# lmb-freiburg/flownet2

Measured on AMD Instinct MI355X. Metric: image-pairs/sec FlowNetC forward at 448x320, higher is better.
Workload: dtype f32

## Files before the change

### flownet2_amd/_lib.py

```python
from __future__ import annotations

import ctypes as C
import os

_HERE = os.path.dirname(os.path.abspath(__file__))
SO_PATH = os.path.join(_HERE, "libflownet2_hip.so")

EXPORTS = [
    "fn2_version", "fn2_last_error_string",
    "fn2_correlation_out_shape", "fn2_correlation_workspace_bytes", "fn2_correlation_forward", "fn2_correlation_forward_fused", "fn2_correlation_backward",
    "fn2_correlation1d_out_shape", "fn2_correlation1d_forward", "fn2_correlation1d_backward",
    "fn2_flow_warp_forward", "fn2_flow_warp_forward_slices", "fn2_flow_warp_backward_workspace_bytes", "fn2_flow_warp_backward",
    "fn2_resample_forward", "fn2_resample_forward_slices",
    "fn2_l1loss_workspace_bytes", "fn2_l1loss_forward", "fn2_l1loss_backward",
    "fn2_l1loss_multi_workspace_bytes", "fn2_l1loss_multi_sync_bytes", "fn2_l1loss_forward_multi", "fn2_l1loss_backward_multi",
    "fn2_channel_norm_forward", "fn2_channel_norm_forward_slices", "fn2_channel_norm_backward",
    "fn2_downsample_forward",
    "fn2_downsample_forward_multi",
    "fn2_predict_flow_conv_workspace_bytes", "fn2_predict_flow_conv_forward", "fn2_upsample_flow_deconv_forward", "fn2_upsample_flow_deconv_forward_into",
    "fn2_predict_flow_conv_backward_supported", "fn2_predict_flow_conv_backward_workspace_bytes", "fn2_predict_flow_conv_backward", "fn2_upsample_flow_deconv_backward_workspace_bytes", "fn2_upsample_flow_deconv_backward",
    "fn2_bias_leaky_relu_forward", "fn2_scale_shift_forward", "fn2_bias_leaky_relu_backward_workspace_bytes", "fn2_bias_leaky_relu_backward", "fn2_bias_leaky_relu_backward_slices", "fn2_bias_leaky_relu_backward_slices2",
    "fn2_conv_k7s2_relu_supported", "fn2_conv_k7s2_relu_forward",
    "fn2_conv_k7s2_wgrad_supported", "fn2_conv_k7s2_wgrad_ksplit", "fn2_conv_k7s2_wgrad_workspace_bytes", "fn2_conv_k7s2_wgrad",
    "fn2_conv_mfma_supported", "fn2_conv_mfma_packed_floats", "fn2_conv_mfma_pack_weights", "fn2_conv_mfma_pack_weights_view", "fn2_conv_mfma_forward",
    "fn2_conv_mfma_num_variants", "fn2_debug_set_conv_variant",
    "fn2_caffemodel_index", "fn2_caffemodel_read_blob", "fn2_hdf5_index", "fn2_hdf5_read_float",
    "fn2_conv_wino_supported", "fn2_conv_wino_packed_floats", "fn2_conv_wino_pack_weights", "fn2_conv_wino_forward",
    "fn2_conv_wino_num_variants", "fn2_debug_set_wino_variant",
    "fn2_conv_plane_supported", "fn2_conv_plane_ksplit", "fn2_conv_plane_workspace_bytes", "fn2_conv_plane_forward",
    "fn2_conv_plane_k_supported", "fn2_conv_plane_k_ksplit", "fn2_conv_plane_k_workspace_bytes", "fn2_conv_plane_k_forward",
    "fn2_conv_plane_num_variants", "fn2_debug_set_plane_variant", "fn2_debug_set_plane_ksplit", "fn2_set_batch_invariant", "fn2_get_batch_invariant",
    "fn2_deconv_plane_supported", "fn2_deconv_plane_ksplit", "fn2_deconv_plane_workspace_bytes", "fn2_deconv_plane_packed_floats",
    "fn2_deconv_plane_pack_weights", "fn2_deconv_plane_pack_weights_k", "fn2_deconv_plane_forward",
    "fn2_tconv_supported", "fn2_tconv_forward", "fn2_tconv_num_variants", "fn2_debug_set_tconv_variant",
    "fn2_debug_set_wgrad_buffers", "fn2_debug_set_wgrad_chunk", "fn2_conv_wgrad_supported", "fn2_conv_wgrad_ksplit", "fn2_conv_wgrad_workspace_bytes", "fn2_conv_wgrad",
    "fn2_conv_bf16x3_supported", "fn2_conv_bf16x3_num_variants", "fn2_debug_set_conv_bf16x3_variant",
    "fn2_conv_route", "fn2_conv_packed_weight_floats", "fn2_conv_pack_weights", "fn2_conv_workspace_bytes", "fn2_conv_forward",
    "fn2_deconv_route", "fn2_deconv_packed_weight_floats", "fn2_deconv_pack_weights", "fn2_deconv_workspace_bytes", "fn2_deconv_forward",
    "fn2_conv_backward_data_route", "fn2_conv_backward_data_packed_weight_floats", "fn2_conv_backward_data_pack_workspace_bytes",
    "fn2_conv_backward_data_pack_weights", "fn2_conv_backward_data_workspace_bytes", "fn2_conv_backward_data_workspace_bytes_with_room", "fn2_conv_backward_data_computed_channels", "fn2_conv_backward_data",
    "fn2_conv_backward_data_masked_supported", "fn2_conv_backward_data_masked", "fn2_conv_backward_weights_bias_fused", "fn2_conv_backward_weights_bias",
    "fn2_conv_backward_weights_supported", "fn2_conv_backward_weights_workspace_bytes", "fn2_conv_backward_weights", "fn2_conv_backward_bias",
    "fn2_im2col_forward", "fn2_col2im_bias_relu_forward", "fn2_col2im_bias_relu_forward_into",
    "fn2_datum_parse", "fn2_datum_float_data", "fn2_datum_serialize",
    "fn2_custom_data_sample_bytes", "fn2_custom_data_encode_sample", "fn2_custom_data_stage_records", "fn2_custom_data_decode_forward",
    "fn2_augmentation_matrix", "fn2_flow_augmentation_forward",
    "fn2_data_augmentation_workspace_bytes", "fn2_data_augmentation_forward",
]


class Fn2Error(RuntimeError):

    def __init__(self, status: int, message: str):
        super().__init__(f"[fn2 status {status}] {message}")
# ... 121 lines not shown
    L.fn2_debug_set_conv_variant.argtypes = [i]
    L.fn2_conv_wino_supported.argtypes = [i] * 5
    L.fn2_conv_wino_packed_floats.argtypes = [i, i]
    L.fn2_conv_wino_packed_floats.restype = sz
    L.fn2_conv_wino_pack_weights.argtypes = [fp, fp, i, i, vp]
    L.fn2_conv_wino_forward.argtypes = [fp, fp, fp, fp] + [i] * 11 + [C.c_float, vp]
    L.fn2_debug_set_wino_variant.argtypes = [i]
    L.fn2_conv_plane_supported.argtypes = [i] * 7
    L.fn2_conv_plane_ksplit.argtypes = [i] * 7
    L.fn2_conv_plane_workspace_bytes.argtypes = [i] * 7
    L.fn2_conv_plane_workspace_bytes.restype = sz
    L.fn2_conv_plane_forward.argtypes = [fp, fp, fp, fp] + [i] * 12 + [C.c_float, vp, sz, vp]
    L.fn2_conv_k7s2_wgrad_supported.argtypes = [i] * 5
    L.fn2_conv_k7s2_wgrad_ksplit.argtypes = [i] * 5
    L.fn2_conv_k7s2_wgrad_workspace_bytes.argtypes = [i] * 5
    L.fn2_conv_k7s2_wgrad_workspace_bytes.restype = sz
    L.fn2_conv_k7s2_wgrad.argtypes = [fp, fp, fp] + [i] * 6 + [vp, sz, vp]
    L.fn2_conv_plane_k_supported.argtypes = [i] * 8
    L.fn2_conv_plane_k_ksplit.argtypes = [i] * 8
    L.fn2_conv_plane_k_workspace_bytes.argtypes = [i] * 8
    L.fn2_conv_plane_k_workspace_bytes.restype = sz
    L.fn2_conv_plane_k_forward.argtypes = [fp, fp, fp, fp] + [i] * 13 + [C.c_float, vp, sz, vp]
    L.fn2_debug_set_plane_variant.argtypes = [i]
    L.fn2_debug_set_plane_ksplit.argtypes = [i]
    L.fn2_set_batch_invariant.argtypes = [i]
    L.fn2_get_batch_invariant.argtypes = []
    L.fn2_tconv_supported.argtypes = [i] * 8
    L.fn2_tconv_forward.argtypes = [fp, fp, fp, fp] + [i] * 14 + [C.c_float, vp]
    L.fn2_debug_set_tconv_variant.argtypes = [i]
    L.fn2_debug_set_wgrad_buffers.argtypes = [i]
    L.fn2_debug_set_wgrad_chunk.argtypes = [i]
    L.fn2_conv_wgrad_supported.argtypes = [i] * 10
    L.fn2_conv_wgrad_ksplit.argtypes = [i] * 10
    L.fn2_conv_wgrad_workspace_bytes.argtypes = [i] * 10
    L.fn2_conv_wgrad_workspace_bytes.restype = sz
    L.fn2_conv_wgrad.argtypes = [fp, fp, fp] + [i] * 15 + [vp, sz, vp]
    L.fn2_deconv_plane_supported.argtypes = [i] * 5
    L.fn2_deconv_plane_ksplit.argtypes = [i] * 5
    L.fn2_deconv_plane_workspace_bytes.argtypes = [i] * 5
    L.fn2_deconv_plane_workspace_bytes.restype = sz
    L.fn2_deconv_plane_packed_floats.argtypes = [i, i]
    L.fn2_deconv_plane_packed_floats.restype = sz
    L.fn2_deconv_plane_pack_weights.argtypes = [fp, fp, i, i, vp]
    L.fn2_deconv_plane_pack_weights_k.argtypes = [fp, fp, i, i, i, vp]
    L.fn2_deconv_plane_forward.argtypes = [fp, fp, fp, fp] + [i] * 10 + [C.c_float, vp, sz, vp]
    L.fn2_caffemodel_index.argtypes = [vp, sz, C.POINTER(CaffemodelEntry), i, C.POINTER(C.c_int)]
# ... 75 lines not shown
```

### flownet2_amd/csrc/conv_plane.hip

```cpp
#include "mfma_tile.hpp"

namespace fn2 {
namespace cp {

using namespace mfma;

constexpr int kNPR = 12;
constexpr int kLdsBytes = 160 * 1024;
constexpr int kSpare = 8;

struct Args {
  const float* in; const float* wp; const float* bias; float* out; float* part;
  int N, Cin, Hin, Win, in_ctot, in_c0;
  int Cout, Hout, Wout, out_ctot, out_c0;
  int pad;
  int P;
  int Wp;
  int img;
  int npb;
  int nig;
  int ng;
  int ksplit;
  int units;
  int ksteps;
  size_t class_stride;
  int rs, cs, wr;
  int band;
  int cap;
  int slots_c, npr;
  int buf;
  unsigned mP, mW, mrs;
  unsigned total;
  float slope; int relu;
};

template <int MODE_, int S_, int MW_, int NP_, int WM_, int WN_, int CQ_, int VEC_, int KS_ = 3>
struct Cfg {
  static constexpr int MODE = MODE_, S = S_, MW = MW_, NP = NP_, WM = WM_, WN = WN_, CQ = CQ_, VEC = VEC_, KS = KS_;
  static constexpr int NCLS = MODE == 1 ? 4 : 1;
  static constexpr int NW = NCLS * WM * WN, THREADS = 64 * NW;
  static constexpr int TAP = MODE == 1 ? 2 : KS;
  static constexpr int PADL = VEC == 4 ? 4 : (KS_ == 5 ? 2 : 1);
  static constexpr int KSC = CQ * TAP * TAP;
  static constexpr int NBUFA = KS_ == 5 ? 5 : (KSC % 9 == 0 && KSC > 9) ? 9 : (KSC % 8 == 0) ? 8 : (KSC % 4 == 0) ? 4 : 3;
  static constexpr int CAP = 16 * NP * WN;
  static_assert(KSC % NBUFA == 0, "ring phase must repeat per chunk");
  static_assert(NBUFA - 1 <= kSpare, "prefetch distance");
  static_assert(MODE == 0 || S == 1, "the deconvolution reads its input at stride 1");
  static_assert(KS == 3 || ((KS == 4 || KS == 5) && MODE == 0 && S == 2), "tap classes: 3x3 / 1, 3x3 / 2, 4x4 / 2, 5x5 / 2");
};

__device__ __forceinline__ int fastdiv(int q, int d, unsigned m) { return d == 1 ? q : (int)__umulhi((unsigned)q, m); }
inline unsigned magic_for(int d) { return d <= 1 ? 0u : (unsigned)(((1ull << 32) + (unsigned)d - 1) / (unsigned)d); }

template <class K>
__device__ __forceinline__ void stage_chunk(__amdgpu_buffer_rsrc_t rs, const unsigned (&voff)[kNPR], const Args& a, unsigned dst, int wave,
                                            unsigned chunk_off, unsigned plane_bytes, unsigned img_bytes, int nimg) {
  const int planes = nimg * 4 * K::CQ;
  const int last = a.slots_c - 64;
  for (int pl = wave; pl < planes; pl += K::NW) {
    const int il = pl / (4 * K::CQ), ch = pl % (4 * K::CQ);
    const unsigned soff = __builtin_amdgcn_readfirstlane(chunk_off + (unsigned)il * img_bytes + (unsigned)ch * plane_bytes);
    const unsigned d0 = __builtin_amdgcn_readfirstlane(dst + 4u * (unsigned)(pl * a.cs));
#pragma unroll
    for (int j = 0; j < kNPR; ++j) {
      if (j < a.npr) {
        const int s0 = 64 * j < last ? 64 * j : last;
        __builtin_amdgcn_raw_ptr_buffer_load_lds(rs, (lds_ptr_t)(uintptr_t)(d0 + 4u * K::VEC * (unsigned)s0), 4 * K::VEC, voff[j], soff, 0, 0);
      }
    }
  }
}

template <class K>
__global__ void __launch_bounds__(K::THREADS)
conv_plane(Args a) {
  extern __shared__ __attribute__((aligned(16))) float smem[];
  constexpr int S = K::S, MW = K::MW, NP = K::NP, TAP = K::TAP;
  unsigned t;
  if (!xcd_task(blockIdx.x, a.total, t)) return;
  const int g = __builtin_amdgcn_readfirstlane((int)(t % a.ng)); t /= a.ng;
  const int pb = __builtin_amdgcn_readfirstlane((int)(t % a.npb)); t /= a.npb;
  const int ig = __builtin_amdgcn_readfirstlane((int)(t % a.nig));
  const int kp = __builtin_amdgcn_readfirstlane((int)(t / a.nig));

  const int tid = threadIdx.x, lane = tid & 63;
  const int wave = __builtin_amdgcn_readfirstlane(tid >> 6);
  const int cls = wave % K::NCLS, w2 = wave / K::NCLS;
  const int py = cls >> 1, px = cls & 1;
  const int wm = w2 % K::WM, wn = w2 / K::WM;
  const int n0 = ig * a.img;
  const int nimg = a.N - n0 < a.img ? a.N - n0 : a.img;

  const int u0 = __builtin_amdgcn_readfirstlane((int)((long long)kp * a.units / a.ksplit));
  const int u1 = __builtin_amdgcn_readfirstlane((int)((long long)(kp + 1) * a.units / a.ksplit));
  const int chunk0 = u0 * (2 / K::CQ), nchunks = (u1 - u0) * (2 / K::CQ);

  const int yblk = a.band ? fastdiv(pb * a.cap, a.Wp, a.mW) : 0;
  const int yorg = (K::MODE == 0 ? S * yblk : yblk) - a.pad;

  const size_t plane = (size_t)a.Hin * a.Win;
  const unsigned plane_bytes = 4u * (unsigned)plane, img_bytes = plane_bytes * (unsigned)a.in_ctot;
  const __amdgpu_buffer_rsrc_t rs = __builtin_amdgcn_make_buffer_rsrc(
      const_cast<float*>(a.in + ((size_t)n0 * a.in_ctot + a.in_c0) * plane), 0,
      (unsigned)(img_bytes * (unsigned)(nimg - 1) + plane_bytes * (unsigned)a.Cin), kRsrcWord3);
  unsigned voff[kNPR];
#pragma unroll
  for (int j = 0; j < kNPR; ++j) {
    voff[j] = kOOB;
    if (j < a.npr) {
      const int last = a.slots_c - 64;
      const int d = K::VEC * ((64 * j < last ? 64 * j : last) + lane);
      const int row = fastdiv(d, a.rs, a.mrs), col = d - row * a.rs;
      const int yi = yorg + row, xi = col - K::PADL;
      if (row < a.wr && yi >= 0 && yi < a.Hin && xi >= 0 && xi < a.Win) voff[j] = 4u * (unsigned)(yi * a.Win + xi);
    }
  }
  const unsigned lds_base = (unsigned)(uintptr_t)(lds_ptr_t)smem;
  const unsigned chunk_bytes = 4u * K::CQ * plane_bytes;

  const int kq = lane >> 4;
  const int tile0 = NP * (pb * K::WN + wn);
  const int lim = nimg * a.P;
  int base[NP];
#pragma unroll
  for (int p = 0; p < NP; ++p) {
    int q = 16 * (tile0 + p) + (lane & 15);
    if (q >= lim) q = 16 * tile0 < lim ? 16 * tile0 : 0;
    const int il = fastdiv(q, a.P, a.mP), rem = q - il * a.P;
    const int y = fastdiv(rem, a.Wp, a.mW), x = rem - y * a.Wp;
    if constexpr (K::MODE == 0) base[p] = (il * 4 * K::CQ + kq) * a.cs + (S * (y - yblk)) * a.rs + S * x + K::PADL - a.pad;
    else base[p] = (il * 4 * K::CQ + kq) * a.cs + (y - yblk + py) * a.rs + x + K::PADL - 1 + px;
  }
  using WV = typename WVec<MW>::T;
  const int cg0 = (g * K::WM + wm) * MW;
  const float* wl = weight_lane(a.wp + (size_t)cls * a.class_stride, cg0, a.ksteps, lane) + (size_t)chunk0 * K::KSC * 256;

  f32x4 acc[MW][NP];
#pragma unroll
  for (int j = 0; j < MW; ++j)
#pragma unroll
    for (int p = 0; p < NP; ++p) acc[j][p] = f32x4{0.f, 0.f, 0.f, 0.f};

  WV wreg[K::NBUFA];
  stage_chunk<K>(rs, voff, a, lds_base, wave, (unsigned)chunk0 * chunk_bytes, plane_bytes, img_bytes, nimg);
#pragma unroll
  for (int i = 0; i < K::NBUFA - 1; ++i) wreg[i] = weight_load<MW>(wl, i);

  for (int c = 0; c < nchunks; ++c) {
    const int buf = c & 1;
    wait_vmcnt<K::NBUFA - 1>();
    __builtin_amdgcn_s_barrier();
    if (c + 1 < nchunks)
      stage_chunk<K>(rs, voff, a, lds_base + 4u * (unsigned)((buf ^ 1) * a.buf), wave, (unsigned)(chunk0 + c + 1) * chunk_bytes, plane_bytes, img_bytes, nimg);
    const float* win = smem + buf * a.buf;
    const int ks0 = c * K::KSC;
    constexpr int NSTEP = K::CQ * TAP;
    float bb[2][TAP][NP];
    auto lds_step = [&](int st, float (&b)[TAP][NP]) {
      const float* wk = win + ((st / TAP) * 4 * a.cs + (st % TAP) * a.rs);
#pragma unroll
      for (int kx = 0; kx < TAP; ++kx)
#pragma unroll
        for (int p = 0; p < NP; ++p) b[kx][p] = wk[base[p] + kx];
    };
    lds_step(0, bb[0]);
    __builtin_amdgcn_sched_barrier(0);
#pragma unroll
    for (int st = 0; st < NSTEP; ++st) {
      const float* wkn = win + (((st + 1) / TAP) * 4 * a.cs + ((st + 1) % TAP) * a.rs);
#pragma unroll
      for (int kx = 0; kx < TAP; ++kx) {
        const int ks = st * TAP + kx;
        wreg[(ks + K::NBUFA - 1) % K::NBUFA] = weight_load<MW>(wl, ks0 + ks + K::NBUFA - 1);
        const WV w = wreg[ks % K::NBUFA];
#pragma unroll
        for (int p = 0; p < NP; ++p) {
#pragma unroll
          for (int j = 0; j < MW; ++j)
            acc[j][p] = __builtin_amdgcn_mfma_f32_16x16x4f32(bb[st & 1][kx][p], wget<MW>(w, j), acc[j][p], 0, 0, 0);
          if (st + 1 < NSTEP) bb[(st + 1) & 1][kx][p] = wkn[base[p] + kx];
          __builtin_amdgcn_sched_barrier(0);
        }
      }
    }
  }

  const bool final_pass = a.ksplit == 1;
  const int Po = a.Hout * a.Wout;
  float* dst = final_pass ? a.out : a.part + (size_t)kp * a.N * a.Cout * Po;
  const int ctot = final_pass ? a.out_ctot : a.Cout, c0 = final_pass ? a.out_c0 : 0;
#pragma unroll
  for (int p = 0; p < NP; ++p) {
    const int q0 = 16 * (tile0 + p) + 4 * (lane >> 4);
    if (q0 >= lim) continue;
    const int il = fastdiv(q0, a.P, a.mP), pix = q0 - il * a.P;
#pragma unroll
    for (int j = 0; j < MW; ++j) {
      const int co = 16 * (cg0 + j) + (lane & 15);
      const float bv = (final_pass && a.bias) ? a.bias[co] : 0.f;
      f32x4 v = acc[j][p];
      if (final_pass) v = bias_relu4(v, bv, a.relu, a.slope);
      if constexpr (K::MODE == 0) {
        float* o = dst + ((size_t)(n0 + il) * ctot + c0 + co) * a.P + pix;
        if (pix + 3 < a.P && (a.P & 3) == 0) *reinterpret_cast<f32x4*>(o) = v;
        else {
          int il2 = il, pix2 = pix;
#pragma unroll
          for (int r = 0; r < 4; ++r) {
            if (q0 + r < lim) dst[((size_t)(n0 + il2) * ctot + c0 + co) * a.P + pix2] = v[r];
// ... 57 lines not shown
    tile[col * ROW + c * T + t] = (ci0 + c < Cin) ? w[((size_t)(ci0 + c) * Cout + co0) * T + e] : 0.f;
  }
  __syncthreads();
  const int j = threadIdx.x & 3, lane = threadIdx.x >> 2;
  const float* trow = tile + (16 * j + (lane & 15)) * ROW + (lane >> 4) * T;
#pragma unroll
  for (int cls = 0; cls < 4; ++cls) {
    const int py = cls >> 1, px = cls & 1;
    float* dst = wp + (((size_t)cls * ngrp + grp) * kalloc + (size_t)8 * u) * 256 + threadIdx.x;
#pragma unroll
    for (int k = 0; k < 8; ++k) {
      const int q = k >> 2, ta = (k >> 1) & 1, tb = k & 1;
      const int ky = py == 0 ? (ta == 0 ? 3 : 1) : (ta == 0 ? 2 : 0), kx = px == 0 ? (tb == 0 ? 3 : 1) : (tb == 0 ? 2 : 0);
      dst[k * 256] = (ky < SK && kx < SK) ? trow[4 * q * T + ky * SK + kx] : 0.f;
    }
    if (8 * (u + 1) >= ksteps)
      for (int i = threadIdx.x; i < (kalloc - ksteps) * 256; i += 256) wp[(((size_t)cls * ngrp + grp) * kalloc + ksteps) * 256 + i] = 0.f;
  }
}

struct Variant {
  int mode, s, mw, np, wm, wn, cq, vec, ks;
  int (*fn)(const Args&, hipStream_t);
};

static bool plan(const Variant& v, Args& a) {
  if (a.Cout % (16 * v.mw * v.wm) != 0) return false;
  if (v.vec == 4 && a.Win % 4 != 0) return false;
  const int padl = v.vec == 4 ? 4 : (v.ks == 5 ? 2 : 1);
  const int cap = 16 * v.np * v.wn;
  a.cap = cap;
  int prow = v.mode == 0 ? a.Hout : a.Hin;
  a.band = 0;
  if (a.P > cap) {
    const int span = (cap + a.Wp - 2) / a.Wp + 1;
    if (span < prow) { prow = span; a.band = 1; }
  }
  if (v.mode == 0) {
    const int wr_need = (prow - 1) * v.s + v.ks;
    a.wr = (!a.band && a.Hin + 2 * a.pad < wr_need) ? a.Hin + 2 * a.pad : wr_need;
  } else {
    a.wr = prow + 2;
  }
  const int wc = padl + a.Win + (v.ks == 5 ? 2 : 1);
  a.rs = v.vec == 4 ? cdiv(wc, 4) * 4 : wc;
  const int plane_dw = a.wr * a.rs < 64 * v.vec ? 64 * v.vec : a.wr * a.rs;
  a.cs = up_mod(plane_dw, 16, 32);
  a.slots_c = a.cs / v.vec;
  a.npr = cdiv(a.slots_c, 64);
  if (a.npr > kNPR) return false;
  int img = 1;
  if (a.P < cap && a.Cin % 8 == 0) {
    img = cap / a.P;
    if (img > a.N) img = a.N;
    while (img > 1 && 2ll * img * 4 * v.cq * a.cs * 4 > kLdsBytes) --img;
  }
  if (2ll * img * 4 * v.cq * a.cs * 4 > kLdsBytes) return false;
  a.img = img;
  a.nig = cdiv(a.N, img);
  a.npb = img == 1 ? cdiv(a.P, cap) : 1;
  a.ng = a.Cout / (16 * v.mw * v.wm);
  a.buf = img * 4 * v.cq * a.cs;
  if ((long long)a.N * a.P >= 65536 || a.cs >= 65536) return false;
  a.mP = magic_for(a.P); a.mW = magic_for(a.Wp); a.mrs = magic_for(a.rs);
  const long long total = (long long)a.ng * a.npb * a.nig * a.ksplit;
  if (total > 0x3fffff00ll) return false;
  a.total = (unsigned)total;
  return true;
}

template <class K>
static int launch(const Args& a, hipStream_t st) {
  const size_t lds = sizeof(float) * 2 * (size_t)a.buf;
  set_dynamic_lds_once<&conv_plane<K>>(kLdsBytes);
  hipLaunchKernelGGL((conv_plane<K>), dim3(8 * ((a.total + 7) / 8)), dim3(K::THREADS), lds, st, a);
  return check_launch("conv_plane_forward");
}

#define FN2_CP_TILES(X, S, VEC) \
  X(0, S, 2, 9, 2, 2, 2, VEC) X(0, S, 2, 5, 2, 2, 2, VEC) X(0, S, 2, 7, 2, 2, 2, VEC) X(0, S, 4, 5, 1, 4, 2, VEC) X(0, S, 2, 9, 1, 4, 1, VEC) \
  X(0, S, 4, 9, 1, 4, 1, VEC) X(0, S, 2, 9, 1, 4, 2, VEC) X(0, S, 4, 4, 2, 2, 2, VEC) \
   \
  X(0, S, 2, 9, 2, 4, 2, VEC) X(0, S, 2, 5, 2, 4, 2, VEC) X(0, S, 2, 5, 4, 2, 2, VEC)
#define FN2_DP_TILES(X, VEC) \
  X(1, 1, 2, 9, 1, 1, 2, VEC) X(1, 1, 2, 9, 1, 1, 1, VEC) X(1, 1, 4, 9, 1, 1, 1, VEC) X(1, 1, 4, 9, 1, 1, 2, VEC) X(1, 1, 2, 5, 1, 1, 2, VEC) \
  X(1, 1, 4, 5, 1, 1, 2, VEC) X(1, 1, 2, 7, 1, 1, 2, VEC) X(1, 1, 4, 7, 1, 1, 1, VEC)
#define FN2_CP_LIST(X) FN2_CP_TILES(X, 1, 1) FN2_CP_TILES(X, 1, 4) FN2_CP_TILES(X, 2, 1) FN2_CP_TILES(X, 2, 4) FN2_DP_TILES(X, 1) FN2_DP_TILES(X, 4)
#define FN2_CP_ROW(MODE, S, MW, NP, WM, WN, CQ, VEC) {MODE, S, MW, NP, WM, WN, CQ, VEC, MODE == 1 ? 4 : 3, &launch<Cfg<MODE, S, MW, NP, WM, WN, CQ, VEC>>},
#define FN2_CP4_TILES(X, VEC) X(2, 9, 2, 2, 2, VEC) X(2, 5, 2, 2, 2, VEC) X(4, 5, 1, 4, 2, VEC) X(2, 5, 2, 4, 2, VEC)
#define FN2_CP4_ROW(MW, NP, WM, WN, CQ, VEC) {0, 2, MW, NP, WM, WN, CQ, VEC, 4, &launch<Cfg<0, 2, MW, NP, WM, WN, CQ, VEC, 4>>},
#define FN2_CP5_TILES(X, VEC) X(2, 9, 2, 2, 1, VEC) X(2, 5, 2, 2, 1, VEC) X(4, 5, 1, 4, 1, VEC) X(2, 9, 1, 4, 1, VEC) X(2, 7, 2, 2, 1, VEC) X(4, 4, 2, 2, 1, VEC)
#define FN2_CP5_ROW(MW, NP, WM, WN, CQ, VEC) {0, 2, MW, NP, WM, WN, CQ, VEC, 5, &launch<Cfg<0, 2, MW, NP, WM, WN, CQ, VEC, 5>>},
static const Variant kVariants[] = {FN2_CP_LIST(FN2_CP_ROW) FN2_CP4_TILES(FN2_CP4_ROW, 1) FN2_CP4_TILES(FN2_CP4_ROW, 4)
                                    FN2_CP5_TILES(FN2_CP5_ROW, 1) FN2_CP5_TILES(FN2_CP5_ROW, 4)};
constexpr int kNumVariants = sizeof(kVariants) / sizeof(kVariants[0]);

int g_forced_variant = -1;
int g_forced_ksplit = 0;

static int ksplit_for(long long mfma_tiles, int units) {
  int k = 1;
  if (g_forced_ksplit > 0) k = g_forced_ksplit;
  else {
    const double want = 14336.0 / (double)mfma_tiles;
    while (k < 16 && (double)k < want) k *= 2;
    if ((double)k > 1.5 * want && k > 1) k /= 2;
  }
  while (k > 1 && k > units) k /= 2;
  return k;
}

static double variant_cost(const Variant& v, const Args& a) {
  const double rounds = (double)((a.total + 255) / 256);
  const double eff = 1.0 / (1.0 + 0.08 * (4.0 / v.mw - 1.0) + 0.02 * (9.0 / v.np - 1.0));
  return rounds * v.mw * v.np / eff;
}

static int forward(Args a, int mode, int stride, int ks, void* workspace, size_t workspace_bytes, const char* what, hipStream_t st) {
  const int Po = a.Hout * a.Wout;
  if (a.ksplit > 1) {
    const size_t need = sizeof(float) * (size_t)a.ksplit * a.N * a.Cout * Po;
    if (!workspace || workspace_bytes < need) return fail(FN2_ERR_WORKSPACE, "%s: workspace of %zu bytes needed", what, need);
    if ((reinterpret_cast<uintptr_t>(workspace) & 15) != 0) return fail(FN2_ERR_UNSUPPORTED, "%s: workspace must be 16-byte aligned", what);
    a.part = static_cast<float*>(workspace);
  }
  auto run = [&](int i) -> int {
    const Variant& v = kVariants[i];
    Args t = a;
    if (v.mode != mode || v.s != stride || v.ks != ks || !plan(v, t)) return FN2_ERR_UNSUPPORTED;
    return v.fn(t, st);
  };
  auto applies = [&](int i) -> bool {
    Args t = a;
    return kVariants[i].mode == mode && kVariants[i].s == stride && kVariants[i].ks == ks && plan(kVariants[i], t);
  };
  auto cost = [&](int i, bool) -> double {
    Args t = a;
    plan(kVariants[i], t);
    return variant_cost(kVariants[i], t);
  };
  static TuneCache cache_conv("conv_plane", kNumVariants), cache_deconv("deconv_plane", kNumVariants);
  const TuneKey key{a.N, a.Cin, a.Hin, a.Win, a.Cout, stride + 16 * ks, a.pad, a.ksplit, a.in_ctot == a.Cin, a.out_ctot == a.Cout};
  Pick p;
  if (const int rc = pick_variant(p, what, g_forced_variant, kNumVariants, false, mode == 0 ? cache_conv : cache_deconv, key, st, applies, cost,
                                  [&](int i, bool) { return run(i); }, [](int) { return false; }))
    return rc;
  if (const int rc = run(p.variant)) return rc;
  if (a.ksplit > 1) {
    const long long total = (long long)a.N * a.Cout * Po;
    if (total >= (1ll << 31)) return fail(FN2_ERR_UNSUPPORTED, "%s: blob too large for the part reduction", what);
    const dim3 rg(blocks_for(total, 256, 4096));
#define FN2_PR(KS_) hipLaunchKernelGGL(plane_reduce<KS_>, rg, dim3(256), 0, st, a.part, a.bias, a.out, a.N, a.Cout, Po, a.out_ctot, a.out_c0, a.ksplit, a.relu, a.slope)
    switch (a.ksplit) {
      case 2: FN2_PR(2); break;
      case 3: FN2_PR(3); break;
      case 4: FN2_PR(4); break;
      case 6: FN2_PR(6); break;
      case 8: FN2_PR(8); break;
      case 12: FN2_PR(12); break;
      case 16: FN2_PR(16); break;
      default: FN2_PR(0); break;
    }
#undef FN2_PR
    return check_launch(what);
  }
  return FN2_OK;
}

static bool supported(const Args& a, int mode, int stride, int ks) {
  for (int i = 0; i < kNumVariants; ++i) {
    Args t = a;
    if (kVariants[i].mode == mode && kVariants[i].s == stride && kVariants[i].ks == ks && plan(kVariants[i], t)) return true;
  }
  return false;
}

}
}

using namespace fn2;

static bool plane_geometry_ok(int N, int Cin, int Hin, int Win, int Cout, int kernel, int stride, int pad) {
  if (N <= 0 || Cin <= 0 || Cin % 8 != 0 || Hin <= 0 || Win <= 0 || Cout <= 0 || Cout % 64 != 0) return false;
  if ((stride != 1 && stride != 2) || pad < 0 || pad > 2) return false;
  if (!((kernel == 3 && pad <= 1) || (kernel == 4 && stride == 2 && pad == 1) || (kernel == 5 && stride == 2 && pad == 2))) return false;
  if (Hin + 2 * pad < kernel || Win + 2 * pad < kernel) return false;
  if ((long long)N * Cin * Hin * Win >= (1ll << 28)) return false;
  return true;
}
// ... 22 lines not shown
  return a.ksplit;
}

FN2_API size_t fn2_conv_plane_k_workspace_bytes(int N, int Cin, int Hin, int Win, int Cout, int kernel, int stride, int pad) {
  if (!plane_geometry_ok(N, Cin, Hin, Win, Cout, kernel, stride, pad)) return 0;
  cp::Args a{};
  fill_args(a, N, Cin, Hin, Win, Cout, kernel, stride, pad);
  return a.ksplit > 1 ? sizeof(float) * (size_t)a.ksplit * N * Cout * a.P : 0;
}

FN2_API int fn2_conv_plane_supported(int N, int Cin, int Hin, int Win, int Cout, int stride, int pad) {
  return fn2_conv_plane_k_supported(N, Cin, Hin, Win, Cout, 3, stride, pad);
}
FN2_API int fn2_conv_plane_ksplit(int N, int Cin, int Hin, int Win, int Cout, int stride, int pad) {
  return fn2_conv_plane_k_ksplit(N, Cin, Hin, Win, Cout, 3, stride, pad);
}
FN2_API size_t fn2_conv_plane_workspace_bytes(int N, int Cin, int Hin, int Win, int Cout, int stride, int pad) {
  return fn2_conv_plane_k_workspace_bytes(N, Cin, Hin, Win, Cout, 3, stride, pad);
}

FN2_API int fn2_debug_set_plane_variant(int v) { cp::g_forced_variant = v; return FN2_OK; }
FN2_API int fn2_debug_set_plane_ksplit(int k) { cp::g_forced_ksplit = k; return FN2_OK; }
FN2_API int fn2_conv_plane_num_variants(void) { return cp::kNumVariants; }

FN2_API int fn2_conv_plane_k_forward(const float* bottom, const float* packed_weight, const float* bias, float* top,
                                     int N, int Cin, int Hin, int Win, int bottom_channels, int bottom_c0,
                                     int Cout, int top_channels, int top_c0, int kernel, int stride, int pad,
                                     int relu, float negative_slope, void* workspace, size_t workspace_bytes, void* stream) {
  if (N < 0) return fail(FN2_ERR_INVALID_ARG, "conv_plane: bad batch");
  if (N == 0) return FN2_OK;
  if (!bottom || !packed_weight || !top) return fail(FN2_ERR_INVALID_ARG, "conv_plane: null blob");
  if (!plane_geometry_ok(N, Cin, Hin, Win, Cout, kernel, stride, pad))
    return fail(FN2_ERR_UNSUPPORTED, "conv_plane: unsupported geometry (N %d, Cin %d, %dx%d, Cout %d, k %d s %d p %d)", N, Cin, Hin, Win, Cout, kernel, stride, pad);
  if (bottom_c0 < 0 || bottom_c0 + Cin > bottom_channels || top_c0 < 0 || top_c0 + Cout > top_channels)
    return fail(FN2_ERR_INVALID_ARG, "conv_plane: channel slice outside the blob");
  if (((reinterpret_cast<uintptr_t>(bottom) | reinterpret_cast<uintptr_t>(top) | reinterpret_cast<uintptr_t>(packed_weight)) & 15) != 0)
    return fail(FN2_ERR_UNSUPPORTED, "conv_plane: blobs must be 16-byte aligned");
  if ((long long)bottom_channels * Hin * Win * 4 * N >= 0x7ffffff0ll) return fail(FN2_ERR_UNSUPPORTED, "conv_plane: bottom blob too large");
  cp::Args a{};
  fill_args(a, N, Cin, Hin, Win, Cout, kernel, stride, pad);
  a.in = bottom; a.wp = packed_weight; a.bias = bias; a.out = top;
  a.in_ctot = bottom_channels; a.in_c0 = bottom_c0; a.out_ctot = top_channels; a.out_c0 = top_c0;
  a.slope = negative_slope; a.relu = relu;
  return cp::forward(a, 0, stride, kernel, workspace, workspace_bytes, "conv_plane", as_stream(stream));
}

// ... 87 lines not shown
```

### flownet2_amd/ops.py

```python
from __future__ import annotations

import ctypes as C

import torch

from . import _lib
from ._lib import CorrParams, L1LossParams, check

MULTIPLY, SUBTRACT = 0, 1
FILL_ZERO, FILL_NAN = 1, 2
NEAREST, LINEAR, CUBIC, AREA = 1, 2, 3, 4


def _stream():
    return C.c_void_p(torch.cuda.current_stream().cuda_stream)


def _chk(t: torch.Tensor, name: str, ndim: int = 4):
    if not isinstance(t, torch.Tensor) or not t.is_cuda:
        raise ValueError(f"{name}: expected a CUDA (HIP) tensor; flownet2_amd has no CPU path")
    if t.dtype != torch.float32:
        raise ValueError(f"{name}: expected float32 (Dtype=float), got {t.dtype}")
    if ndim is not None and t.dim() != ndim:
        raise ValueError(f"{name}: expected {ndim} axes (NCHW), got shape {tuple(t.shape)}")
# ... 855 lines not shown
    check(_lib.lib().fn2_deconv_plane_forward(_ptr(x), _ptr(pw), _ptr(b), _ptr(out), N, Cin, H, W, Ctot, in_c0, Cout, out.shape[1], out_c0,
                                              int(bool(relu)), C.c_float(float(negative_slope)), _ptr(ws if need else None), need, _stream()))
    return out


def set_plane_variant(v: int):
    check(_lib.lib().fn2_debug_set_plane_variant(int(v)))


def set_plane_ksplit(k: int):
    check(_lib.lib().fn2_debug_set_plane_ksplit(int(k)))


def set_batch_invariant(on: bool):
    check(_lib.lib().fn2_set_batch_invariant(1 if on else 0))


def get_batch_invariant() -> bool:
    return bool(_lib.lib().fn2_get_batch_invariant())


def plane_num_variants() -> int:
    return int(_lib.lib().fn2_conv_plane_num_variants())


def set_wino_variant(v: int):
    check(_lib.lib().fn2_debug_set_wino_variant(int(v)))


def wino_num_variants() -> int:
    return int(_lib.lib().fn2_conv_wino_num_variants())


def im2col_forward(x, kernel, pad, stride):
    x = _chk(x, "bottom[0]")
    N, Cc, H, W = x.shape
    Hc, Wc = (H + 2 * pad - kernel) // stride + 1, (W + 2 * pad - kernel) // stride + 1
    col = torch.empty((N, Cc * kernel * kernel, Hc * Wc), device=x.device, dtype=torch.float32)
    check(_lib.lib().fn2_im2col_forward(_ptr(x), _ptr(col), N, Cc, H, W, int(kernel), int(pad), int(stride), _stream()))
    return col


def col2im_bias_relu_forward(col, bias, N, Cc, H, W, kernel, pad, stride, relu=True, negative_slope=0.1, out=None, out_c0=0):
    if not (col.is_cuda and col.dtype == torch.float32 and col.is_contiguous()):
        raise ValueError("col2im: expected a contiguous float32 CUDA (HIP) column blob")
    Hc, Wc = (H + 2 * pad - kernel) // stride + 1, (W + 2 * pad - kernel) // stride + 1
# ... 103 lines not shown
```

### include/flownet2_hip.h

```cpp
#ifndef FLOWNET2_HIP_H_
#define FLOWNET2_HIP_H_

#include <stddef.h>

#ifdef __cplusplus
extern "C" {
#endif

#define FN2_VERSION_MAJOR 0
#define FN2_VERSION_MINOR 1

typedef enum fn2_status {
  FN2_OK = 0,
  FN2_ERR_INVALID_ARG = -1,
  FN2_ERR_UNSUPPORTED = -2,
  FN2_ERR_WORKSPACE = -3,
  FN2_ERR_LAUNCH = -4
} fn2_status;

const char* fn2_version(void);
const char* fn2_last_error_string(void);

enum { FN2_CORR_MULTIPLY = 0, FN2_CORR_SUBTRACT = 1 };

// ... 156 lines not shown
size_t fn2_conv_wino_packed_floats(int Cout, int Cin);
int fn2_conv_wino_pack_weights(const float* weight, float* packed, int Cout, int Cin, void* stream);
int fn2_conv_wino_forward(const float* bottom, const float* packed_weight, const float* bias, float* top,
                          int N, int Cin, int Hin, int Win, int bottom_channels, int bottom_c0,
                          int Cout, int top_channels, int top_c0, int pad, int relu, float negative_slope, void* stream);
int fn2_conv_wino_num_variants(void);
int fn2_debug_set_wino_variant(int variant);

int fn2_conv_plane_supported(int N, int Cin, int Hin, int Win, int Cout, int stride, int pad);
int fn2_conv_plane_ksplit(int N, int Cin, int Hin, int Win, int Cout, int stride, int pad);
size_t fn2_conv_plane_workspace_bytes(int N, int Cin, int Hin, int Win, int Cout, int stride, int pad);
int fn2_conv_plane_forward(const float* bottom, const float* packed_weight, const float* bias, float* top,
                           int N, int Cin, int Hin, int Win, int bottom_channels, int bottom_c0,
                           int Cout, int top_channels, int top_c0, int stride, int pad,
                           int relu, float negative_slope, void* workspace, size_t workspace_bytes, void* stream);
int fn2_conv_plane_k_supported(int N, int Cin, int Hin, int Win, int Cout, int kernel, int stride, int pad);
int fn2_conv_plane_k_ksplit(int N, int Cin, int Hin, int Win, int Cout, int kernel, int stride, int pad);
size_t fn2_conv_plane_k_workspace_bytes(int N, int Cin, int Hin, int Win, int Cout, int kernel, int stride, int pad);
int fn2_conv_plane_k_forward(const float* bottom, const float* packed_weight, const float* bias, float* top,
                             int N, int Cin, int Hin, int Win, int bottom_channels, int bottom_c0,
                             int Cout, int top_channels, int top_c0, int kernel, int stride, int pad,
                             int relu, float negative_slope, void* workspace, size_t workspace_bytes, void* stream);
int fn2_conv_plane_num_variants(void);
int fn2_debug_set_plane_variant(int variant);
int fn2_debug_set_plane_ksplit(int ksplit);
int fn2_set_batch_invariant(int on);
int fn2_get_batch_invariant(void);

int fn2_deconv_plane_supported(int N, int Cin, int Hin, int Win, int Cout);
int fn2_deconv_plane_ksplit(int N, int Cin, int Hin, int Win, int Cout);
size_t fn2_deconv_plane_workspace_bytes(int N, int Cin, int Hin, int Win, int Cout);
size_t fn2_deconv_plane_packed_floats(int Cin, int Cout);
int fn2_deconv_plane_pack_weights(const float* weight, float* packed, int Cin, int Cout, void* stream);
int fn2_deconv_plane_pack_weights_k(const float* weight, float* packed, int Cin, int Cout, int src_kernel, void* stream);
int fn2_deconv_plane_forward(const float* bottom, const float* packed_weight, const float* bias, float* top,
                             int N, int Cin, int Hin, int Win, int bottom_channels, int bottom_c0,
                             int Cout, int top_channels, int top_c0, int relu, float negative_slope,
                             void* workspace, size_t workspace_bytes, void* stream);

typedef struct fn2_conv_desc {
  int N, Cin, Hin, Win;
  int Cout, kernel, stride, pad;
} fn2_conv_desc;
enum { FN2_CONV_ROUTE_NONE = 0, FN2_CONV_ROUTE_DIRECT = 1, FN2_CONV_ROUTE_WINOGRAD = 2, FN2_CONV_ROUTE_PLANE = 3, FN2_CONV_ROUTE_STEM = 4,
       FN2_CONV_ROUTE_HEAD = 5 };
enum { FN2_DECONV_ROUTE_NONE = 0, FN2_DECONV_ROUTE_GEMM = 1, FN2_DECONV_ROUTE_PLANE = 2, FN2_DECONV_ROUTE_HEAD = 3 };
// ... 155 lines not shown
```

Baseline: 3539.

## Add fused-K conv_plane variants reducing split-K parts in LDS within one block

Adds conv_plane variants in which each wave of a block computes one K-split part with its own LDS staging buffer. The partial sums are then reduced through shared memory and written with bias and ReLU, which removes the separate plane_reduce launch and the round trip of partials through global memory. A counted-staging form unrolls the plane loads to a fixed count. The variants are picked by the cost model, which scales fused variants by a fixed gain factor, or by autotuning. In exchange each block uses more LDS, and the grid has fewer blocks.

```diff
diff --git a/flownet2_amd/_lib.py b/flownet2_amd/_lib.py
--- a/flownet2_amd/_lib.py
+++ b/flownet2_amd/_lib.py
@@ -29,7 +29,7 @@
     "fn2_conv_wino_num_variants", "fn2_debug_set_wino_variant",
     "fn2_conv_plane_supported", "fn2_conv_plane_ksplit", "fn2_conv_plane_workspace_bytes", "fn2_conv_plane_forward",
     "fn2_conv_plane_k_supported", "fn2_conv_plane_k_ksplit", "fn2_conv_plane_k_workspace_bytes", "fn2_conv_plane_k_forward",
-    "fn2_conv_plane_num_variants", "fn2_debug_set_plane_variant", "fn2_debug_set_plane_ksplit", "fn2_set_batch_invariant", "fn2_get_batch_invariant",
+    "fn2_conv_plane_num_variants", "fn2_conv_plane_variant_fused_ksplit", "fn2_debug_set_plane_variant", "fn2_debug_set_plane_ksplit", "fn2_set_batch_invariant", "fn2_get_batch_invariant",
     "fn2_deconv_plane_supported", "fn2_deconv_plane_ksplit", "fn2_deconv_plane_workspace_bytes", "fn2_deconv_plane_packed_floats",
     "fn2_deconv_plane_pack_weights", "fn2_deconv_plane_pack_weights_k", "fn2_deconv_plane_forward",
     "fn2_tconv_supported", "fn2_tconv_forward", "fn2_tconv_num_variants", "fn2_debug_set_tconv_variant",
@@ -197,6 +197,7 @@
     L.fn2_conv_plane_k_workspace_bytes.restype = sz
     L.fn2_conv_plane_k_forward.argtypes = [fp, fp, fp, fp] + [i] * 13 + [C.c_float, vp, sz, vp]
     L.fn2_debug_set_plane_variant.argtypes = [i]
+    L.fn2_conv_plane_variant_fused_ksplit.argtypes = [i]
     L.fn2_debug_set_plane_ksplit.argtypes = [i]
     L.fn2_set_batch_invariant.argtypes = [i]
     L.fn2_get_batch_invariant.argtypes = []
diff --git a/flownet2_amd/csrc/conv_plane.hip b/flownet2_amd/csrc/conv_plane.hip
--- a/flownet2_amd/csrc/conv_plane.hip
+++ b/flownet2_amd/csrc/conv_plane.hip
@@ -29,24 +29,28 @@
   int cap;
   int slots_c, npr;
   int buf;
+  int wavebuf;
   unsigned mP, mW, mrs;
   unsigned total;
   float slope; int relu;
 };
 
-template <int MODE_, int S_, int MW_, int NP_, int WM_, int WN_, int CQ_, int VEC_, int KS_ = 3>
+template <int MODE_, int S_, int MW_, int NP_, int WM_, int WN_, int CQ_, int VEC_, int KS_ = 3, int KP_ = 0, int IMGM_ = 0, int NPRM_ = 0>
 struct Cfg {
-  static constexpr int MODE = MODE_, S = S_, MW = MW_, NP = NP_, WM = WM_, WN = WN_, CQ = CQ_, VEC = VEC_, KS = KS_;
+  static constexpr int MODE = MODE_, S = S_, MW = MW_, NP = NP_, WM = WM_, WN = WN_, CQ = CQ_, VEC = VEC_, KS = KS_, KP = KP_, IMGM = IMGM_, NPRM = NPRM_;
   static constexpr int NCLS = MODE == 1 ? 4 : 1;
-  static constexpr int NW = NCLS * WM * WN, THREADS = 64 * NW;
+  static constexpr int NW = KP > 0 ? KP : NCLS * WM * WN, THREADS = 64 * NW;
+  static constexpr int STAGE_STEP = KP > 0 ? 1 : NW;
   static constexpr int TAP = MODE == 1 ? 2 : KS;
   static constexpr int PADL = VEC == 4 ? 4 : (KS_ == 5 ? 2 : 1);
   static constexpr int KSC = CQ * TAP * TAP;
-  static constexpr int NBUFA = KS_ == 5 ? 5 : (KSC % 9 == 0 && KSC > 9) ? 9 : (KSC % 8 == 0) ? 8 : (KSC % 4 == 0) ? 4 : 3;
+  static constexpr int NBUFA = (NPRM_ > 0 && KSC == 9) ? 9 : KS_ == 5 ? 5 : (KSC % 9 == 0 && KSC > 9) ? 9 : (KSC % 8 == 0) ? 8 : (KSC % 4 == 0) ? 4 : 3;
   static constexpr int CAP = 16 * NP * WN;
   static_assert(KSC % NBUFA == 0, "ring phase must repeat per chunk");
   static_assert(NBUFA - 1 <= kSpare, "prefetch distance");
   static_assert(MODE == 0 || S == 1, "the deconvolution reads its input at stride 1");
+  static_assert(KP == 0 || (MODE == 0 && WM == 1 && WN == 1 && KP >= 2 && KP <= 16), "fused K: one wave per K part, convolution only");
+  static_assert(NPRM == 0 || (KP > 0 && IMGM > 0 && NPRM <= kNPR), "counted staging is a fused-K form");
   static_assert(KS == 3 || ((KS == 4 || KS == 5) && MODE == 0 && S == 2), "tap classes: 3x3 / 1, 3x3 / 2, 4x4 / 2, 5x5 / 2");
 };
 
@@ -58,7 +62,7 @@
                                             unsigned chunk_off, unsigned plane_bytes, unsigned img_bytes, int nimg) {
   const int planes = nimg * 4 * K::CQ;
   const int last = a.slots_c - 64;
-  for (int pl = wave; pl < planes; pl += K::NW) {
+  for (int pl = wave; pl < planes; pl += K::STAGE_STEP) {
     const int il = pl / (4 * K::CQ), ch = pl % (4 * K::CQ);
     const unsigned soff = __builtin_amdgcn_readfirstlane(chunk_off + (unsigned)il * img_bytes + (unsigned)ch * plane_bytes);
     const unsigned d0 = __builtin_amdgcn_readfirstlane(dst + 4u * (unsigned)(pl * a.cs));
@@ -73,20 +77,49 @@
 }
 
 template <class K>
+__device__ __forceinline__ void stage_chunk_counted(__amdgpu_buffer_rsrc_t rs, const unsigned (&voff)[kNPR], const Args& a, unsigned dst,
+                                                    unsigned chunk_off, unsigned plane_bytes, unsigned img_bytes, int nimg) {
+  const int last = a.slots_c - 64;
+#pragma unroll
+  for (int pl = 0; pl < K::IMGM * 4 * K::CQ; ++pl) {
+    const int ch = pl % (4 * K::CQ);
+    const int il = pl / (4 * K::CQ) < nimg ? pl / (4 * K::CQ) : nimg - 1;
+    const unsigned soff = __builtin_amdgcn_readfirstlane(chunk_off + (unsigned)il * img_bytes + (unsigned)ch * plane_bytes);
+    const unsigned d0 = __builtin_amdgcn_readfirstlane(dst + 4u * (unsigned)((il * 4 * K::CQ + ch) * a.cs));
+#pragma unroll
+    for (int j = 0; j < K::NPRM; ++j) {
+      const int s0 = 64 * j < last ? 64 * j : last;
+      __builtin_amdgcn_raw_ptr_buffer_load_lds(rs, (lds_ptr_t)(uintptr_t)(d0 + 4u * K::VEC * (unsigned)s0), 4 * K::VEC, voff[j], soff, 0, 0);
+    }
+  }
+}
+
+template <class K>
 __global__ void __launch_bounds__(K::THREADS)
 conv_plane(Args a) {
   extern __shared__ __attribute__((aligned(16))) float smem[];
   constexpr int S = K::S, MW = K::MW, NP = K::NP, TAP = K::TAP;
+  constexpr bool FUSED = K::KP > 0, COUNTED = K::NPRM > 0;
+  const int tid = threadIdx.x, lane = tid & 63;
+  const int wave = __builtin_amdgcn_readfirstlane(tid >> 6);
   unsigned t;
   if (!xcd_task(blockIdx.x, a.total, t)) return;
-  const int g = __builtin_amdgcn_readfirstlane((int)(t % a.ng)); t /= a.ng;
-  const int pb = __builtin_amdgcn_readfirstlane((int)(t % a.npb)); t /= a.npb;
-  const int ig = __builtin_amdgcn_readfirstlane((int)(t % a.nig));
-  const int kp = __builtin_amdgcn_readfirstlane((int)(t / a.nig));
-
-  const int tid = threadIdx.x, lane = tid & 63;
-  const int wave = __builtin_amdgcn_readfirstlane(tid >> 6);
-  const int cls = wave % K::NCLS, w2 = wave / K::NCLS;
+  int g, pb, ig, kp;
+  if constexpr (FUSED) {
+    pb = __builtin_amdgcn_readfirstlane((int)(t % a.npb)); t /= a.npb;
+    ig = __builtin_amdgcn_readfirstlane((int)(t % a.nig));
+    g = __builtin_amdgcn_readfirstlane((int)(t / a.nig));
+    kp = wave;
+  } else {
+    g = __builtin_amdgcn_readfirstlane((int)(t % a.ng)); t /= a.ng;
+    pb = __builtin_amdgcn_readfirstlane((int)(t % a.npb)); t /= a.npb;
+    ig = __builtin_amdgcn_readfirstlane((int)(t % a.nig));
+    kp = __builtin_amdgcn_readfirstlane((int)(t / a.nig));
+  }
+
+  const int wsub = FUSED ? 0 : wave;
+  const int swave = FUSED ? 0 : wave;
+  const int cls = wsub % K::NCLS, w2 = wsub / K::NCLS;
   const int py = cls >> 1, px = cls & 1;
   const int wm = w2 % K::WM, wn = w2 / K::WM;
   const int n0 = ig * a.img;
@@ -108,7 +141,7 @@
 #pragma unroll
   for (int j = 0; j < kNPR; ++j) {
     voff[j] = kOOB;
-    if (j < a.npr) {
+    if (COUNTED ? j < K::NPRM : j < a.npr) {
       const int last = a.slots_c - 64;
       const int d = K::VEC * ((64 * j < last ? 64 * j : last) + lane);
       const int row = fastdiv(d, a.rs, a.mrs), col = d - row * a.rs;
@@ -116,7 +149,8 @@
       if (row < a.wr && yi >= 0 && yi < a.Hin && xi >= 0 && xi < a.Win) voff[j] = 4u * (unsigned)(yi * a.Win + xi);
     }
   }
-  const unsigned lds_base = (unsigned)(uintptr_t)(lds_ptr_t)smem;
+  float* const wsmem = FUSED ? smem + (size_t)wave * a.wavebuf : smem;
+  const unsigned lds_base = (unsigned)(uintptr_t)(lds_ptr_t)wsmem;
   const unsigned chunk_bytes = 4u * K::CQ * plane_bytes;
 
   const int kq = lane >> 4;
@@ -143,17 +177,20 @@
     for (int p = 0; p < NP; ++p) acc[j][p] = f32x4{0.f, 0.f, 0.f, 0.f};
 
   WV wreg[K::NBUFA];
-  stage_chunk<K>(rs, voff, a, lds_base, wave, (unsigned)chunk0 * chunk_bytes, plane_bytes, img_bytes, nimg);
+  stage_chunk<K>(rs, voff, a, lds_base, swave, (unsigned)chunk0 * chunk_bytes, plane_bytes, img_bytes, nimg);
 #pragma unroll
   for (int i = 0; i < K::NBUFA - 1; ++i) wreg[i] = weight_load<MW>(wl, i);
 
   for (int c = 0; c < nchunks; ++c) {
     const int buf = c & 1;
     wait_vmcnt<K::NBUFA - 1>();
-    __builtin_amdgcn_s_barrier();
-    if (c + 1 < nchunks)
-      stage_chunk<K>(rs, voff, a, lds_base + 4u * (unsigned)((buf ^ 1) * a.buf), wave, (unsigned)(chunk0 + c + 1) * chunk_bytes, plane_bytes, img_bytes, nimg);
-    const float* win = smem + buf * a.buf;
+    if constexpr (!FUSED) __builtin_amdgcn_s_barrier();
+    if constexpr (COUNTED)
+      stage_chunk_counted<K>(rs, voff, a, lds_base + 4u * (unsigned)((buf ^ 1) * a.buf), (unsigned)(chunk0 + (c + 1 < nchunks ? c + 1 : c)) * chunk_bytes,
+                             plane_bytes, img_bytes, nimg);
+    else if (c + 1 < nchunks)
+      stage_chunk<K>(rs, voff, a, lds_base + 4u * (unsigned)((buf ^ 1) * a.buf), swave, (unsigned)(chunk0 + c + 1) * chunk_bytes, plane_bytes, img_bytes, nimg);
+    const float* win = wsmem + buf * a.buf;
     const int ks0 = c * K::KSC;
     constexpr int NSTEP = K::CQ * TAP;
     float bb[2][TAP][NP];
@@ -186,6 +223,39 @@
     }
   }
 
+  if constexpr (FUSED) {
+    if constexpr (COUNTED) wait_vmcnt<0>();
+#pragma unroll
+    for (int j = 0; j < MW; ++j)
+#pragma unroll
+      for (int p = 0; p < NP; ++p) *reinterpret_cast<f32x4*>(wsmem + ((j * NP + p) * 64 + lane) * 4) = acc[j][p];
+    __syncthreads();
+    for (int i = tid; i < MW * NP * 64; i += K::THREADS) {
+      const int tl = i >> 6, l = i & 63, j = tl / NP, p = tl - j * NP;
+      f32x4 v[K::KP];
+#pragma unroll
+      for (int k = 0; k < K::KP; ++k) v[k] = *reinterpret_cast<const f32x4*>(smem + (size_t)k * a.wavebuf + 4 * i);
+      f32x4 s = v[0];
+#pragma unroll
+      for (int k = 1; k < K::KP; ++k) s += v[k];
+      const int q0 = 16 * (tile0 + p) + 4 * (l >> 4);
+      if (q0 >= lim) continue;
+      const int il = fastdiv(q0, a.P, a.mP), pix = q0 - il * a.P;
+      const int co = 16 * (cg0 + j) + (l & 15);
+      s = bias_relu4(s, a.bias ? a.bias[co] : 0.f, a.relu, a.slope);
+      float* o = a.out + ((size_t)(n0 + il) * a.out_ctot + a.out_c0 + co) * a.P + pix;
+      if (pix + 3 < a.P && (a.P & 3) == 0) *reinterpret_cast<f32x4*>(o) = s;
+      else {
+        int il2 = il, pix2 = pix;
+#pragma unroll
+        for (int r = 0; r < 4; ++r) {
+          if (q0 + r < lim) a.out[((size_t)(n0 + il2) * a.out_ctot + a.out_c0 + co) * a.P + pix2] = s[r];
+          if (++pix2 == a.P) { pix2 = 0; ++il2; }
+        }
+      }
+    }
+    return;
+  }
   const bool final_pass = a.ksplit == 1;
   const int Po = a.Hout * a.Wout;
   float* dst = final_pass ? a.out : a.part + (size_t)kp * a.N * a.Cout * Po;
@@ -289,9 +359,13 @@
 struct Variant {
   int mode, s, mw, np, wm, wn, cq, vec, ks;
   int (*fn)(const Args&, hipStream_t);
+  int kp;
+  int imgm, nprm;
 };
 
 static bool plan(const Variant& v, Args& a) {
+  if (v.kp > 0 && a.ksplit != v.kp) return false;
+  const int nwin = v.kp > 0 ? v.kp : 1;
   if (a.Cout % (16 * v.mw * v.wm) != 0) return false;
   if (v.vec == 4 && a.Win % 4 != 0) return false;
   const int padl = v.vec == 4 ? 4 : (v.ks == 5 ? 2 : 1);
@@ -315,22 +389,28 @@
   a.cs = up_mod(plane_dw, 16, 32);
   a.slots_c = a.cs / v.vec;
   a.npr = cdiv(a.slots_c, 64);
-  if (a.npr > kNPR) return false;
+  if (a.npr > kNPR || (v.nprm > 0 && a.npr > v.nprm)) return false;
   int img = 1;
   if (a.P < cap && a.Cin % 8 == 0) {
     img = cap / a.P;
     if (img > a.N) img = a.N;
-    while (img > 1 && 2ll * img * 4 * v.cq * a.cs * 4 > kLdsBytes) --img;
-  }
-  if (2ll * img * 4 * v.cq * a.cs * 4 > kLdsBytes) return false;
+    if (v.nprm > 0 && img > v.imgm) img = v.imgm;
+    while (img > 1 && 2ll * nwin * img * 4 * v.cq * a.cs * 4 > kLdsBytes) --img;
+  }
+  if (2ll * nwin * img * 4 * v.cq * a.cs * 4 > kLdsBytes) return false;
   a.img = img;
   a.nig = cdiv(a.N, img);
   a.npb = img == 1 ? cdiv(a.P, cap) : 1;
   a.ng = a.Cout / (16 * v.mw * v.wm);
   a.buf = img * 4 * v.cq * a.cs;
+  a.wavebuf = 0;
+  if (v.kp > 0) {
+    a.wavebuf = 2 * a.buf > v.mw * v.np * 256 ? 2 * a.buf : v.mw * v.np * 256;
+    if (4ll * v.kp * a.wavebuf > kLdsBytes) return false;
+  }
   if ((long long)a.N * a.P >= 65536 || a.cs >= 65536) return false;
   a.mP = magic_for(a.P); a.mW = magic_for(a.Wp); a.mrs = magic_for(a.rs);
-  const long long total = (long long)a.ng * a.npb * a.nig * a.ksplit;
+  const long long total = (long long)a.ng * a.npb * a.nig * (v.kp > 0 ? 1 : a.ksplit);
   if (total > 0x3fffff00ll) return false;
   a.total = (unsigned)total;
   return true;
@@ -338,7 +418,7 @@
 
 template <class K>
 static int launch(const Args& a, hipStream_t st) {
-  const size_t lds = sizeof(float) * 2 * (size_t)a.buf;
+  const size_t lds = sizeof(float) * (K::KP > 0 ? (size_t)K::KP * a.wavebuf : 2 * (size_t)a.buf);
   set_dynamic_lds_once<&conv_plane<K>>(kLdsBytes);
   hipLaunchKernelGGL((conv_plane<K>), dim3(8 * ((a.total + 7) / 8)), dim3(K::THREADS), lds, st, a);
   return check_launch("conv_plane_forward");
@@ -358,8 +438,14 @@
 #define FN2_CP4_ROW(MW, NP, WM, WN, CQ, VEC) {0, 2, MW, NP, WM, WN, CQ, VEC, 4, &launch<Cfg<0, 2, MW, NP, WM, WN, CQ, VEC, 4>>},
 #define FN2_CP5_TILES(X, VEC) X(2, 9, 2, 2, 1, VEC) X(2, 5, 2, 2, 1, VEC) X(4, 5, 1, 4, 1, VEC) X(2, 9, 1, 4, 1, VEC) X(2, 7, 2, 2, 1, VEC) X(4, 4, 2, 2, 1, VEC)
 #define FN2_CP5_ROW(MW, NP, WM, WN, CQ, VEC) {0, 2, MW, NP, WM, WN, CQ, VEC, 5, &launch<Cfg<0, 2, MW, NP, WM, WN, CQ, VEC, 5>>},
+#define FN2_FK_TILES(X, S) X(16, 1, 5, 1, S) X(8, 2, 5, 1, S) X(4, 2, 5, 2, S) X(2, 4, 5, 1, S)
+#define FN2_FK_ROW(KP, MW, NP, CQ, S) {0, S, MW, NP, 1, 1, CQ, 1, 3, &launch<Cfg<0, S, MW, NP, 1, 1, CQ, 1, 3, KP>>, KP, 0, 0},
+#define FN2_FKC_LIST(X) X(8, 1, 9, 1, 1, 1, 1, 4) X(8, 2, 5, 1, 1, 1, 1, 3) X(8, 2, 5, 1, 2, 4, 1, 3)
+#define FN2_FKC_ROW(KP, MW, NP, CQ, S, VEC, IMGM, NPRM) {0, S, MW, NP, 1, 1, CQ, VEC, 3, &launch<Cfg<0, S, MW, NP, 1, 1, CQ, VEC, 3, KP, IMGM, NPRM>>, KP, IMGM, NPRM},
 static const Variant kVariants[] = {FN2_CP_LIST(FN2_CP_ROW) FN2_CP4_TILES(FN2_CP4_ROW, 1) FN2_CP4_TILES(FN2_CP4_ROW, 4)
-                                    FN2_CP5_TILES(FN2_CP5_ROW, 1) FN2_CP5_TILES(FN2_CP5_ROW, 4)};
+                                    FN2_CP5_TILES(FN2_CP5_ROW, 1) FN2_CP5_TILES(FN2_CP5_ROW, 4)
+                                    FN2_FK_TILES(FN2_FK_ROW, 1) FN2_FK_TILES(FN2_FK_ROW, 2)
+                                    FN2_FKC_LIST(FN2_FKC_ROW)};
 constexpr int kNumVariants = sizeof(kVariants) / sizeof(kVariants[0]);
 
 int g_forced_variant = -1;
@@ -377,9 +463,11 @@
   return k;
 }
 
+constexpr double kFusedGain = 0.83;
 static double variant_cost(const Variant& v, const Args& a) {
   const double rounds = (double)((a.total + 255) / 256);
   const double eff = 1.0 / (1.0 + 0.08 * (4.0 / v.mw - 1.0) + 0.02 * (9.0 / v.np - 1.0));
+  if (v.kp > 0) return rounds * v.mw * v.np * (v.kp > 4 ? v.kp / 4.0 : 1.0) / eff * kFusedGain;
   return rounds * v.mw * v.np / eff;
 }
 
@@ -391,11 +479,30 @@
     if ((reinterpret_cast<uintptr_t>(workspace) & 15) != 0) return fail(FN2_ERR_UNSUPPORTED, "%s: workspace must be 16-byte aligned", what);
     a.part = static_cast<float*>(workspace);
   }
+  auto reduce = [&]() -> int {
+    const long long total = (long long)a.N * a.Cout * Po;
+    if (total >= (1ll << 31)) return fail(FN2_ERR_UNSUPPORTED, "%s: blob too large for the part reduction", what);
+    const dim3 rg(blocks_for(total, 256, 4096));
+#define FN2_PR(KS_) hipLaunchKernelGGL(plane_reduce<KS_>, rg, dim3(256), 0, st, a.part, a.bias, a.out, a.N, a.Cout, Po, a.out_ctot, a.out_c0, a.ksplit, a.relu, a.slope)
+    switch (a.ksplit) {
+      case 2: FN2_PR(2); break;
+      case 3: FN2_PR(3); break;
+      case 4: FN2_PR(4); break;
+      case 6: FN2_PR(6); break;
+      case 8: FN2_PR(8); break;
+      case 12: FN2_PR(12); break;
+      case 16: FN2_PR(16); break;
+      default: FN2_PR(0); break;
+    }
+#undef FN2_PR
+    return check_launch(what);
+  };
   auto run = [&](int i) -> int {
     const Variant& v = kVariants[i];
     Args t = a;
     if (v.mode != mode || v.s != stride || v.ks != ks || !plan(v, t)) return FN2_ERR_UNSUPPORTED;
-    return v.fn(t, st);
+    if (const int rc = v.fn(t, st)) return rc;
+    return (a.ksplit > 1 && v.kp == 0) ? reduce() : FN2_OK;
   };
   auto applies = [&](int i) -> bool {
     Args t = a;
@@ -412,26 +519,7 @@
   if (const int rc = pick_variant(p, what, g_forced_variant, kNumVariants, false, mode == 0 ? cache_conv : cache_deconv, key, st, applies, cost,
                                   [&](int i, bool) { return run(i); }, [](int) { return false; }))
     return rc;
-  if (const int rc = run(p.variant)) return rc;
-  if (a.ksplit > 1) {
-    const long long total = (long long)a.N * a.Cout * Po;
-    if (total >= (1ll << 31)) return fail(FN2_ERR_UNSUPPORTED, "%s: blob too large for the part reduction", what);
-    const dim3 rg(blocks_for(total, 256, 4096));
-#define FN2_PR(KS_) hipLaunchKernelGGL(plane_reduce<KS_>, rg, dim3(256), 0, st, a.part, a.bias, a.out, a.N, a.Cout, Po, a.out_ctot, a.out_c0, a.ksplit, a.relu, a.slope)
-    switch (a.ksplit) {
-      case 2: FN2_PR(2); break;
-      case 3: FN2_PR(3); break;
-      case 4: FN2_PR(4); break;
-      case 6: FN2_PR(6); break;
-      case 8: FN2_PR(8); break;
-      case 12: FN2_PR(12); break;
-      case 16: FN2_PR(16); break;
-      default: FN2_PR(0); break;
-    }
-#undef FN2_PR
-    return check_launch(what);
-  }
-  return FN2_OK;
+  return run(p.variant);
 }
 
 static bool supported(const Args& a, int mode, int stride, int ks) {
@@ -500,6 +588,7 @@
 FN2_API int fn2_debug_set_plane_variant(int v) { cp::g_forced_variant = v; return FN2_OK; }
 FN2_API int fn2_debug_set_plane_ksplit(int k) { cp::g_forced_ksplit = k; return FN2_OK; }
 FN2_API int fn2_conv_plane_num_variants(void) { return cp::kNumVariants; }
+FN2_API int fn2_conv_plane_variant_fused_ksplit(int v) { return (v >= 0 && v < cp::kNumVariants) ? cp::kVariants[v].kp : 0; }
 
 FN2_API int fn2_conv_plane_k_forward(const float* bottom, const float* packed_weight, const float* bias, float* top,
                                      int N, int Cin, int Hin, int Win, int bottom_channels, int bottom_c0,
diff --git a/flownet2_amd/ops.py b/flownet2_amd/ops.py
--- a/flownet2_amd/ops.py
+++ b/flownet2_amd/ops.py
@@ -901,6 +901,10 @@
 
 def plane_num_variants() -> int:
     return int(_lib.lib().fn2_conv_plane_num_variants())
+
+
+def plane_variant_fused_parts(v: int) -> int:
+    return int(_lib.lib().fn2_conv_plane_variant_fused_ksplit(int(v)))
 
 
 def set_wino_variant(v: int):
diff --git a/include/flownet2_hip.h b/include/flownet2_hip.h
--- a/include/flownet2_hip.h
+++ b/include/flownet2_hip.h
@@ -202,6 +202,7 @@
                              int Cout, int top_channels, int top_c0, int kernel, int stride, int pad,
                              int relu, float negative_slope, void* workspace, size_t workspace_bytes, void* stream);
 int fn2_conv_plane_num_variants(void);
+int fn2_conv_plane_variant_fused_ksplit(int variant);
 int fn2_debug_set_plane_variant(int variant);
 int fn2_debug_set_plane_ksplit(int ksplit);
 int fn2_set_batch_invariant(int on);
```

New measurement: 3565, median of 6. No clear change (+0.7%).
